# td-kwj-zp2023/webgpu-msm-bls12-377

Hardware: AMD Instinct MI355X
Metric: ms per 2^20 BLS12-377 G1 MSM (lower is better)
Workload: dtype u32 (29-bit limbs, 64-bit accumulate)

## Files before the change

webgpu-msm-bls12-377_amd/csrc/curves.hpp:

```cpp
#pragma once
#include <hip/hip_runtime.h>

#include "common.hpp"
#include "fp64_host.hpp"
#include "g1_xyzz.hpp"
#include "te377.hpp"

namespace msm377 {
namespace {


__device__ __forceinline__ void load_words16(const uint32_t* __restrict__ p, uint32_t* w, int nvec) {
  const uint4* s = reinterpret_cast<const uint4*>(p);
#pragma unroll
  for (int k = 0; k < nvec; k++) {
    uint4 v = s[k];
    w[4 * k + 0] = v.x;
    w[4 * k + 1] = v.y;
    w[4 * k + 2] = v.z;
    w[4 * k + 3] = v.w;
  }
}

struct G1Dev {
  static constexpr uint32_t REC_WORDS = 32;
  static constexpr bool HAS_QUAD = true;
  static constexpr uint32_t RAW_WORDS = 24;
  static constexpr uint32_t PT_WORDS = 52;
  static constexpr uint32_t COORD_WORDS = 16;
  static constexpr uint32_t BKT_WORDS = 4 * COORD_WORDS;
  static constexpr uint32_t OUT_WORDS = 48;
  static constexpr uint32_t RECORD_TAG = 0;
  static constexpr int MADD_PRODUCTS = 10;
  static constexpr int FORM_ID = MSM377_STAGE_FORM_XYZZ;
  using F = Fp;
  static constexpr uint32_t NL = 13, NW32 = 12;
  static __device__ __forceinline__ Fp::El to64() { return Fp::from_const(G1Consts::TO64); }
  using Base = G1Affine;
  using Pt = G1XYZZ;
  static __device__ __forceinline__ bool convert(const uint32_t* raw, uint32_t* rec) {
    Fp::El x = Fp::to_mont(Fp::from_words<12>(raw));
    Fp::El y = Fp::to_mont(Fp::from_words<12>(raw + 12));
#pragma unroll
    for (int j = 0; j < 13; j++) {
      rec[j] = x.l[j];
      rec[13 + j] = y.l[j];
    }
#pragma unroll
    for (int j = 26; j < 32; j++) rec[j] = 0;
    return false;
  }
  static __device__ __forceinline__ Base load_base(const uint32_t* __restrict__ bases, uint32_t idx) {
    uint32_t w[28];
    load_words16(bases + (size_t)idx * REC_WORDS, w, 7);
    Base p;
#pragma unroll
    for (int j = 0; j < 13; j++) {
      p.x.l[j] = w[j];
      p.y.l[j] = w[13 + j];
    }
    return p;
  }
  static __device__ __forceinline__ bool is_bad(const Pt&) { return false; }
  static __device__ __forceinline__ bool is_stored_identity(const Pt& p) { return G1::is_identity(p); }
  static __device__ __forceinline__ Pt identity() { return G1::identity(); }
  static __device__ __forceinline__ Pt madd(const Pt& a, const Base& q, bool negq) { return G1::madd(a, q, negq); }
  static __device__ __forceinline__ Pt first(const Base& q, bool negq) { return G1::madd(G1::identity(), q, negq); }
  static __device__ __forceinline__ Pt add(const Pt& a, const Pt& b) { return G1::add(a, b); }
  static __device__ __forceinline__ void to_words(const Pt& p, uint32_t* w) {
#pragma unroll
    for (int j = 0; j < 13; j++) {
      w[j] = p.x.l[j];
      w[13 + j] = p.y.l[j];
      w[26 + j] = p.zz.l[j];
      w[39 + j] = p.zzz.l[j];
    }
  }
  static __device__ __forceinline__ Pt from_words(const uint32_t* w) {
    Pt p;
#pragma unroll
    for (int j = 0; j < 13; j++) {
      p.x.l[j] = w[j];
      p.y.l[j] = w[13 + j];
      p.zz.l[j] = w[26 + j];
      p.zzz.l[j] = w[39 + j];
    }
    return p;
  }
};

struct EdDev {
  static constexpr uint32_t REC_WORDS = 32;
  static constexpr bool HAS_QUAD = true;
  static constexpr uint32_t RAW_WORDS = 16;
  static constexpr uint32_t PT_WORDS = 36;
  static constexpr uint32_t COORD_WORDS = 12;
  static constexpr uint32_t BKT_WORDS = 4 * COORD_WORDS;
  static constexpr uint32_t OUT_WORDS = 32;
  static constexpr uint32_t RECORD_TAG = 0;
  static constexpr int MADD_PRODUCTS = 7;
  static constexpr int FORM_ID = -1;
  using F = Fq;
  static constexpr uint32_t NL = 9, NW32 = 8;
  static __device__ __forceinline__ Fq::El to64() { return Fq::from_const(EdConsts::TO64); }
  using Base = EdLazy::ABase;
  using Pt = EdLazy::Ext;
  static __device__ __forceinline__ bool convert(const uint32_t* raw, uint32_t* rec) {
    Fq::El x = Fq::to_mont(Fq::from_words<8>(raw));
    Fq::El y = Fq::to_mont(Fq::from_words<8>(raw + 8));
    const Ed::Base b = Ed::make_base(x, y);
#pragma unroll
    for (int j = 0; j < 9; j++) {
      rec[j] = b.ymx.l[j];
      rec[9 + j] = b.ypx.l[j];
      rec[18 + j] = b.kt.l[j];
    }
#pragma unroll
    for (int j = 27; j < 32; j++) rec[j] = 0;
    return false;
  }
  static __device__ __forceinline__ Base load_base(const uint32_t* __restrict__ bases, uint32_t idx) {
    uint32_t w[28];
    load_words16(bases + (size_t)idx * REC_WORDS, w, 7);
    Base p;
#pragma unroll
    for (int j = 0; j < 9; j++) {
      p.ymx.l[j] = w[j];
      p.ypx.l[j] = w[9 + j];
      p.kt.l[j] = w[18 + j];
    }
    return p;
  }

  static __device__ __forceinline__ bool is_bad(const Pt&) { return false; }
  static __device__ __forceinline__ bool is_stored_identity(const Pt& p) { return Fq::is_zero(p.x) && Fq::eq(p.y, p.z); }
  static __device__ __forceinline__ Pt identity() { return EdLazy::identity(); }
  static __device__ __forceinline__ Pt madd(const Pt& a, const Base& q, bool negq) { return EdLazy::madd_affine(a, q, negq); }
  static __device__ __forceinline__ Pt first(const Base& q, bool negq) { return EdLazy::madd_affine(EdLazy::identity(), q, negq); }
  static __device__ __forceinline__ Pt add(const Pt& a, const Pt& b) { return EdLazy::add(a, b); }
  static __device__ __forceinline__ void to_words(const Pt& p, uint32_t* w) {
#pragma unroll
    for (int j = 0; j < 9; j++) {
      w[j] = p.x.l[j];
      w[9 + j] = p.y.l[j];
      w[18 + j] = p.t.l[j];
      w[27 + j] = p.z.l[j];
    }
  }
  static __device__ __forceinline__ Pt from_words(const uint32_t* w) {
    Pt p;
#pragma unroll
    for (int j = 0; j < 9; j++) {
      p.x.l[j] = w[j];
      p.y.l[j] = w[9 + j];
      p.t.l[j] = w[18 + j];
      p.z.l[j] = w[27 + j];
    }
    return p;
  }
};

struct TeDev {
  static constexpr uint32_t REC_WORDS = 64;
  static constexpr bool HAS_QUAD = true;
  static constexpr uint32_t RAW_WORDS = 24;
  static constexpr uint32_t PT_WORDS = 52;
  static constexpr uint32_t COORD_WORDS = 16;
  static constexpr uint32_t BKT_WORDS = 4 * COORD_WORDS;
  static constexpr uint32_t OUT_WORDS = 48;
  static constexpr uint32_t RECORD_TAG = TE_RECORD_TAG;
  static constexpr int MADD_PRODUCTS = 8;
  static constexpr int FORM_ID = MSM377_STAGE_FORM_TE;
  using F = Fp;
  static constexpr uint32_t NL = 13, NW32 = 12;
  static __device__ __forceinline__ Fp::El to64() { return Fp::from_const(G1Consts::TO64); }
  using Base = Te377::PBase;
  using Pt = Te377::Ext;
  using Pt_K = G1Consts;
  static __device__ __forceinline__ bool convert(const uint32_t* raw, uint32_t* rec) {
    const Base b = Te377::from_wire(raw, raw + 12, false);
#pragma unroll
    for (int j = 0; j < 13; j++) {
      rec[j] = b.ymx.l[j];
      rec[13 + j] = b.ypx.l[j];
      rec[26 + j] = b.kt.l[j];
      rec[39 + j] = b.z2.l[j];
    }
#pragma unroll
    for (int j = 52; j < 64; j++) rec[j] = 0;
    return Fp::is_zero(b.z2);
  }
  static __device__ __forceinline__ Base load_base(const uint32_t* __restrict__ bases, uint32_t idx) {
    uint32_t w[52];
    load_words16(bases + (size_t)idx * REC_WORDS, w, 13);
    Base p;
#pragma unroll
    for (int j = 0; j < 13; j++) {
      p.ymx.l[j] = w[j];
      p.ypx.l[j] = w[13 + j];
      p.kt.l[j] = w[26 + j];
      p.z2.l[j] = w[39 + j];
    }
    return p;
  }
  static __device__ __forceinline__ bool is_bad(const Pt& p) { return Te377::is_bad(p); }
  static __device__ __forceinline__ bool is_stored_identity(const Pt& p) { return Fp::is_zero(p.x) && Fp::eq(p.y, p.z); }
  static __device__ __forceinline__ Pt identity() { return Te377::identity(); }
  static __device__ __forceinline__ Pt madd(const Pt& a, const Base& q, bool negq) { return Te377::madd(a, q, negq); }
  static __device__ __forceinline__ Pt first(const Base& q, bool negq) { return Te377::from_base(q, negq); }
  static __device__ __forceinline__ Pt add(const Pt& a, const Pt& b) { return Te377::add(a, b); }
  static __device__ __forceinline__ void to_words(const Pt& p, uint32_t* w) {
#pragma unroll
    for (int j = 0; j < 13; j++) {
      w[j] = p.x.l[j];
      w[13 + j] = p.y.l[j];
      w[26 + j] = p.t.l[j];
      w[39 + j] = p.z.l[j];
    }
  }
  static __device__ __forceinline__ Pt from_words(const uint32_t* w) {
    Pt p;
#pragma unroll
    for (int j = 0; j < 13; j++) {
      p.x.l[j] = w[j];
      p.y.l[j] = w[13 + j];
      p.t.l[j] = w[26 + j];
      p.z.l[j] = w[39 + j];
    }
    return p;
  }
};

struct TeAffBase {
  static constexpr uint32_t REC_WORDS = 40;
  static constexpr int MADD_PRODUCTS = 7;
  using Base = Te377::ABase;
  using Pt = Te377::Ext;
  static __device__ __forceinline__ Base load_base(const uint32_t* __restrict__ bases, uint32_t idx) {
    uint32_t w[40];
    load_words16(bases + (size_t)idx * REC_WORDS, w, 10);
    Base p;
#pragma unroll
    for (int j = 0; j < 13; j++) {
      p.ymx.l[j] = w[j];
      p.ypx.l[j] = w[13 + j];
      p.kt.l[j] = w[26 + j];
    }
    return p;
  }
  static __device__ __forceinline__ Pt madd(const Pt& a, const Base& q, bool negq) { return Te377::madd_affine(a, q, negq); }
  static __device__ __forceinline__ Pt first(const Base& q, bool negq) { return Te377::from_base_affine(q, negq); }
};

template <class CV>
__device__ __forceinline__ typename CV::Pt load_record(const uint32_t* __restrict__ p) {
  uint32_t w[CV::PT_WORDS];
#pragma unroll
  for (uint32_t c = 0; c < 4; c++) {
    const uint4* s = reinterpret_cast<const uint4*>(p + c * CV::COORD_WORDS);
#pragma unroll
    for (uint32_t k = 0; k < CV::NL / 4; k++) {
      const uint4 v = s[k];
      w[c * CV::NL + 4 * k + 0] = v.x;
      w[c * CV::NL + 4 * k + 1] = v.y;
      w[c * CV::NL + 4 * k + 2] = v.z;
      w[c * CV::NL + 4 * k + 3] = v.w;
    }
    static_assert(CV::NL % 4 == 1, "one limb beyond the 16-byte groups");
    w[c * CV::NL + CV::NL - 1] = p[c * CV::COORD_WORDS + CV::NL - 1];
  }
  return CV::from_words(w);
}
template <class CV>
__device__ __forceinline__ void store_coord(uint32_t* __restrict__ slot, const uint32_t* l) {
  uint4* d = reinterpret_cast<uint4*>(slot);
#pragma unroll
  for (uint32_t k = 0; k < CV::NL / 4; k++) d[k] = make_uint4(l[4 * k], l[4 * k + 1], l[4 * k + 2], l[4 * k + 3]);
  d[CV::NL / 4] = make_uint4(l[CV::NL - 1], 0u, 0u, 0u);
  static_assert(CV::COORD_WORDS == (CV::NL / 4 + 1) * 4, "slot = limbs rounded up to 16 bytes");
}
template <class CV>
__device__ __forceinline__ void store_record(uint32_t* __restrict__ p, const typename CV::Pt& r) {
  uint32_t w[CV::PT_WORDS];
  CV::to_words(r, w);
#pragma unroll
  for (uint32_t c = 0; c < 4; c++) store_coord<CV>(p + c * CV::COORD_WORDS, w + c * CV::NL);
}
template <class CV>
__device__ __forceinline__ uint32_t* bucket_ptr(uint32_t* b, uint32_t L, uint32_t ws, uint32_t t) { return b + (((size_t)ws << L) + t) * CV::BKT_WORDS; }
template <class CV>
__device__ __forceinline__ const uint32_t* bucket_ptr(const uint32_t* b, uint32_t L, uint32_t ws, uint32_t t) { return b + (((size_t)ws << L) + t) * CV::BKT_WORDS; }
template <class CV>
__device__ __forceinline__ typename CV::Pt load_bucket(const uint32_t* __restrict__ b, uint32_t L, uint32_t ws, uint32_t t) {
  return load_record<CV>(bucket_ptr<CV>(b, L, ws, t));
}
template <class CV>
__device__ __forceinline__ void store_bucket(uint32_t* __restrict__ b, uint32_t L, uint32_t ws, uint32_t t, const typename CV::Pt& r) {
  store_record<CV>(bucket_ptr<CV>(b, L, ws, t), r);
}

static_assert(G1Dev::REC_WORDS == G1_REC_WORDS, "common.hpp sizes the base table with it");

}
}
```

webgpu-msm-bls12-377_amd/csrc/field29.hpp:

```cpp
#pragma once
#include <stdint.h>

#if defined(__HIPCC__)
#include <hip/hip_runtime.h>
#define MSM_HD __host__ __device__ __forceinline__
#else
#define MSM_HD inline __attribute__((always_inline))
#endif

#include "consts_gen.hpp"

namespace msm377 {

constexpr int LB = 29;
constexpr uint32_t LMASK = (1u << LB) - 1u;

template <int N>
struct Limbs {
  uint32_t l[N];
};

template <class C>
struct Field {
  static constexpr int N = C::NL;
  static constexpr int RS = C::RS;
  using Consts = C;
  using El = Limbs<N>;

  static MSM_HD El zero() {
    El r;
#pragma unroll
    for (int j = 0; j < N; j++) r.l[j] = 0;
    return r;
  }
  static MSM_HD El from_const(const uint32_t (&c)[N]) {
    El r;
#pragma unroll
    for (int j = 0; j < N; j++) r.l[j] = c[j];
    return r;
  }
  static MSM_HD El one() { return from_const(C::ONE); }

  static MSM_HD bool is_zero(const El& a) {
    uint32_t acc = 0;
#pragma unroll
    for (int j = 0; j < N; j++) acc |= a.l[j];
    return acc == 0;
  }
  static MSM_HD bool eq(const El& a, const El& b) {
    uint32_t acc = 0;
#pragma unroll
    for (int j = 0; j < N; j++) acc |= (a.l[j] ^ b.l[j]);
    return acc == 0;
  }
  static MSM_HD El select(bool c, const El& a, const El& b) {
    El r;
#pragma unroll
    for (int j = 0; j < N; j++) r.l[j] = c ? a.l[j] : b.l[j];
    return r;
  }

  static MSM_HD El reduce_once(const El& x) {
    El d;
    int32_t bw = 0;
#pragma unroll
    for (int j = 0; j < N - 1; j++) {
      int32_t v = (int32_t)x.l[j] - (int32_t)C::MOD[j] + bw;
      d.l[j] = (uint32_t)v & LMASK;
      bw = v >> 31;
    }
    int32_t top = (int32_t)x.l[N - 1] - (int32_t)C::MOD[N - 1] + bw;
    d.l[N - 1] = (uint32_t)top;
    return select(top < 0, x, d);
  }

  static MSM_HD El add(const El& a, const El& b) {
    El s;
    uint32_t c = 0;
#pragma unroll
    for (int j = 0; j < N - 1; j++) {
      uint32_t v = a.l[j] + b.l[j] + c;
      s.l[j] = v & LMASK;
      c = v >> LB;
    }
    s.l[N - 1] = a.l[N - 1] + b.l[N - 1] + c;
    return reduce_once(s);
  }
  static MSM_HD El dbl(const El& a) { return add(a, a); }

  static MSM_HD El sub(const El& a, const El& b) {
    El d, e;
    int32_t bw = 0, c2 = 0;
#pragma unroll
    for (int j = 0; j < N - 1; j++) {
      int32_t v = (int32_t)a.l[j] - (int32_t)b.l[j];
      int32_t v1 = v + bw;
      d.l[j] = (uint32_t)v1 & LMASK;
      bw = v1 >> 31;
      int32_t v2 = v + (int32_t)C::MOD[j] + c2;
      e.l[j] = (uint32_t)v2 & LMASK;
      c2 = v2 >> LB;
    }
    int32_t v = (int32_t)a.l[N - 1] - (int32_t)b.l[N - 1];
    int32_t top = v + bw;
    d.l[N - 1] = (uint32_t)top;
    e.l[N - 1] = (uint32_t)(v + (int32_t)C::MOD[N - 1] + c2);
    return select(top < 0, e, d);
  }

  static MSM_HD El neg(const El& a) {
    El r;
    int32_t bw = 0;
    uint32_t nz = 0;
#pragma unroll
    for (int j = 0; j < N; j++) {
      nz |= a.l[j];
      int32_t v = (int32_t)C::MOD[j] - (int32_t)a.l[j] + bw;
      r.l[j] = (j < N - 1) ? ((uint32_t)v & LMASK) : (uint32_t)v;
      bw = v >> 31;
    }
    return select(nz != 0, r, a);
  }
  static MSM_HD El cneg(const El& a, bool c) { return select(c, neg(a), a); }


  static MSM_HD El mul_lz(const El& a, const El& b) {
    uint64_t t[N];
#pragma unroll
    for (int j = 0; j < N; j++) t[j] = 0;
#pragma unroll
    for (int i = 0; i < RS; i++) {
      if (i < N) {
#pragma unroll
        for (int j = 0; j < N; j++) t[j] += (uint64_t)a.l[i] * b.l[j];
      }
      uint32_t q = (0u - (uint32_t)t[0]) & LMASK;
      uint64_t carry = (t[0] + q) >> LB;
#pragma unroll
      for (int j = 1; j < N; j++) t[j] += (uint64_t)q * C::MOD[j];
      t[1] += carry;
#pragma unroll
      for (int j = 0; j < N - 1; j++) t[j] = t[j + 1];
      t[N - 1] = 0;
    }
    El r;
#pragma unroll
    for (int j = 0; j < N - 1; j++) {
      r.l[j] = (uint32_t)t[j] & LMASK;
      t[j + 1] += t[j] >> LB;
    }
    r.l[N - 1] = (uint32_t)t[N - 1];
    return r;
  }

  static MSM_HD El mul_add_mul_lz(const El& a, const El& b, const El& e, const El& d) {
    uint64_t t[N];
#pragma unroll
    for (int j = 0; j < N; j++) t[j] = 0;
#pragma unroll
    for (int i = 0; i < RS; i++) {
      if (i < N) {
#pragma unroll
        for (int j = 0; j < N; j++) t[j] += (uint64_t)a.l[i] * b.l[j];
#pragma unroll
        for (int j = 0; j < N; j++) t[j] += (uint64_t)e.l[i] * d.l[j];
      }
      uint32_t q = (0u - (uint32_t)t[0]) & LMASK;
      uint64_t carry = (t[0] + q) >> LB;
#pragma unroll
      for (int j = 1; j < N; j++) t[j] += (uint64_t)q * C::MOD[j];
      t[1] += carry;
#pragma unroll
      for (int j = 0; j < N - 1; j++) t[j] = t[j + 1];
      t[N - 1] = 0;
    }
    El r;
#pragma unroll
    for (int j = 0; j < N - 1; j++) {
      r.l[j] = (uint32_t)t[j] & LMASK;
      t[j + 1] += t[j] >> LB;
    }
    r.l[N - 1] = (uint32_t)t[N - 1];
    return r;
  }

  static MSM_HD El sqr_lz(const El& a) {
    uint64_t t[RS + N];
#pragma unroll
    for (int j = 0; j < RS + N; j++) t[j] = 0;
#pragma unroll
    for (int i = 0; i < N; i++) {
      t[2 * i] += (uint64_t)a.l[i] * a.l[i];
      const uint32_t a2 = a.l[i] << 1;
#pragma unroll
      for (int j = i + 1; j < N; j++) t[i + j] += (uint64_t)a2 * a.l[j];
    }
#pragma unroll
    for (int i = 0; i < RS; i++) {
      uint32_t q = (0u - (uint32_t)t[i]) & LMASK;
      uint64_t carry = (t[i] + q) >> LB;
#pragma unroll
      for (int j = 1; j < N; j++) t[i + j] += (uint64_t)q * C::MOD[j];
      t[i + 1] += carry;
    }
    El r;
#pragma unroll
    for (int j = 0; j < N - 1; j++) {
      r.l[j] = (uint32_t)t[RS + j] & LMASK;
      t[RS + j + 1] += t[RS + j] >> LB;
    }
    r.l[N - 1] = (uint32_t)t[RS + N - 1];
    return r;
  }

  static MSM_HD El mul(const El& a, const El& b) { return reduce_once(mul_lz(a, b)); }
  static MSM_HD El sqr(const El& a) { return reduce_once(sqr_lz(a)); }
  static MSM_HD El mul_sub_mul(const El& a, const El& b, const El& c, const El& d) {
    const El r = mul_add_mul_lz(a, b, neg(c), d);
    return RS > N ? reduce_once(r) : reduce_once(reduce_once(r));
  }


  static MSM_HD El add_kp_sub(const El& a, const uint32_t (&K)[N], const El& b) {
    El r;
#pragma unroll
    for (int j = 0; j < N; j++) r.l[j] = a.l[j] + K[j] - b.l[j];
    return r;
  }
  static MSM_HD El add_lz(const El& a, const El& b) {
    El r;
#pragma unroll
    for (int j = 0; j < N; j++) r.l[j] = a.l[j] + b.l[j];
    return r;
  }
  static MSM_HD El kp_sub(const uint32_t (&K)[N], const El& b) {
    El r;
#pragma unroll
    for (int j = 0; j < N; j++) r.l[j] = K[j] - b.l[j];
    return r;
  }
  static MSM_HD El add_kp_sub_sub2(const El& a, const uint32_t (&K)[N], const El& b, const El& b2) {
    El r;
#pragma unroll
    for (int j = 0; j < N; j++) r.l[j] = a.l[j] + K[j] - b.l[j] - 2u * b2.l[j];
    return r;
  }
  static MSM_HD El norm(const El& a) {
    El r;
    uint32_t c = 0;
#pragma unroll
    for (int j = 0; j < N - 1; j++) {
      const uint32_t v = a.l[j] + c;
      r.l[j] = v & LMASK;
      c = v >> LB;
    }
    r.l[N - 1] = a.l[N - 1] + c;
    return r;
  }
  static MSM_HD El csub(const El& x, const uint32_t (&m)[N]) {
    El d;
    int32_t bw = 0;
#pragma unroll
    for (int j = 0; j < N - 1; j++) {
      const int32_t v = (int32_t)x.l[j] - (int32_t)m[j] + bw;
      d.l[j] = (uint32_t)v & LMASK;
      bw = v >> 31;
    }
    const int64_t top = (int64_t)x.l[N - 1] - (int64_t)m[N - 1] + bw;
    d.l[N - 1] = (uint32_t)top;
    return select(top < 0, x, d);
  }
  static MSM_HD El canon(const El& x) { return csub(csub(csub(x, C::MOD4), C::MOD2), C::MOD); }

  static MSM_HD El to_mont(const El& a) { return mul(a, from_const(C::R2)); }
  static MSM_HD El from_mont(const El& a) {
    El o = zero();
    o.l[0] = 1;
    return mul(a, o);
  }

  template <int NW>
  static MSM_HD El from_words(const uint32_t* w) {
    El r;
#pragma unroll
    for (int j = 0; j < N; j++) {
      const int bit = LB * j, wi = bit >> 5, off = bit & 31;
      uint32_t v = 0;
      if (wi < NW) v = w[wi] >> off;
      if (off > 32 - LB && wi + 1 < NW) v |= w[wi + 1] << (32 - off);
      r.l[j] = v & LMASK;
    }
    return r;
  }
  template <int NW>
  static MSM_HD void to_words(const El& a, uint32_t* w) {
#pragma unroll
    for (int k = 0; k < NW; k++) w[k] = 0;
#pragma unroll
    for (int j = 0; j < N; j++) {
      const int bit = LB * j, wi = bit >> 5, off = bit & 31;
      if (wi < NW) w[wi] |= a.l[j] << off;
      if (off > 32 - LB && wi + 1 < NW) w[wi + 1] |= a.l[j] >> (32 - off);
    }
  }
};

using Fp = Field<G1Consts>;
using Fq = Field<EdConsts>;

template <class F, int NW>
MSM_HD typename F::El fe_pow(const typename F::El& a, const uint32_t* e) {
  typename F::El r = F::one();
  for (int i = NW * 32 - 1; i >= 0; i--) {
    r = F::sqr(r);
    if ((e[i >> 5] >> (i & 31)) & 1u) r = F::mul(r, a);
  }
  return r;
}

}
```

webgpu-msm-bls12-377_amd/csrc/kernels/accumulate.hpp:

```cpp
#pragma once
#include "../curves.hpp"
#include "reduce.hpp"

namespace msm377 {
namespace {



__device__ __forceinline__ const uint32_t* row_bounds(const uint32_t* __restrict__ row_ptr, uint32_t L, uint32_t ws, uint32_t t) {
  return row_ptr + (size_t)ws * ((1u << L) + 2) + t + 1;
}
__device__ __forceinline__ uint32_t row_len(const uint32_t* __restrict__ row_ptr, uint32_t L, uint32_t row) {
  const int at = (int)(row + 2 * (row >> L) + 1);
  return row_ptr[at + 1] - row_ptr[at];
}

struct RowSplit {
  uint32_t nseg, seglen, lastlen;
};
__device__ __forceinline__ RowSplit row_split(uint32_t len, uint32_t SEG) {
  RowSplit r;
  if (len <= SEG) {
    r.nseg = 1;
    r.seglen = r.lastlen = len;
    return r;
  }
  const uint32_t parts = (len + SEG - 1) / SEG;
  r.seglen = (len + parts - 1) / parts;
  r.nseg = (len + r.seglen - 1) / r.seglen;
  r.lastlen = len - (r.nseg - 1) * r.seglen;
  return r;
}

__global__ void __launch_bounds__(1024) k_work_hist(const uint32_t* __restrict__ row_ptr, uint32_t L, uint32_t rows, uint32_t SEG, uint32_t* __restrict__ work_hist,
                                                   uint32_t* __restrict__ row_ovf_base, uint32_t* __restrict__ counters ,
                                                   uint32_t* __restrict__ split_rows) {
  __shared__ uint32_t lh[SEG_BINS];
  __shared__ uint32_t blk[4];
  const uint32_t tid = threadIdx.x, row = blockIdx.x * 1024 + tid;
  if (tid < SEG_BINS) lh[tid] = 0;
  if (tid < 2) blk[tid] = 0;
  __syncthreads();
  RowSplit sp = {1, 0, 0};
  uint32_t my_split = 0, my_ovf = 0;
  if (row < rows) {
    sp = row_split(row_len(row_ptr, L, row), SEG);
    atomicAdd(&lh[sp.lastlen], 1u);
    if (sp.nseg > 1) {
      atomicAdd(&lh[sp.seglen], sp.nseg - 1);
      my_split = atomicAdd(&blk[0], 1u);
      my_ovf = atomicAdd(&blk[1], sp.nseg - 1);
    }
  }
  __syncthreads();
  if (tid < SEG_BINS && lh[tid]) atomicAdd(&work_hist[tid], lh[tid]);
  if (tid == 0 && blk[0]) {
    blk[2] = atomicAdd(&counters[0], blk[0]);
    blk[3] = atomicAdd(&counters[1], blk[1]);
  }
  __syncthreads();
  if (sp.nseg > 1) {
    row_ovf_base[row] = blk[3] + my_ovf;
    split_rows[blk[2] + my_split] = row;
  }
}

__global__ void __launch_bounds__(1024) k_work_scatter(const uint32_t* __restrict__ row_ptr, uint32_t L, uint32_t rows, uint32_t SEG,
                                                      const uint32_t* __restrict__ work_hist, uint32_t* __restrict__ cursor, uint32_t* __restrict__ total,
                                                      WorkItem* __restrict__ work) {
  __shared__ uint32_t lh[SEG_BINS];
  __shared__ uint32_t lbase[SEG_BINS];
  __shared__ uint32_t gh[SEG_BINS];
  const uint32_t tid = threadIdx.x, row = blockIdx.x * 1024 + tid;
  if (tid < SEG_BINS) {
    lh[tid] = 0;
    gh[tid] = work_hist[tid];
  }
  __syncthreads();
  uint32_t first = 0;
  if (tid < SEG_BINS) {
    for (uint32_t b = tid + 1; b < SEG_BINS; b++) first += gh[b];
    if (tid == 0 && blockIdx.x == 0) *total = first + gh[0];
  }
  RowSplit sp = {0, 0, 0};
  uint32_t rank_full = 0, rank_last = 0;
  if (row < rows) {
    sp = row_split(row_len(row_ptr, L, row), SEG);
    if (sp.nseg > 1) rank_full = atomicAdd(&lh[sp.seglen], sp.nseg - 1);
    rank_last = atomicAdd(&lh[sp.lastlen], 1u);
  }
  __syncthreads();
  if (tid < SEG_BINS && lh[tid]) lbase[tid] = first + atomicAdd(&cursor[tid], lh[tid]);
  __syncthreads();
  if (row < rows) {
    for (uint32_t s = 0; s + 1 < sp.nseg; s++) work[lbase[sp.seglen] + rank_full + s] = WorkItem{row, s};
    work[lbase[sp.lastlen] + rank_last] = WorkItem{row, sp.nseg - 1};
  }
}

template <class CV, int OCC, class BP = CV, int PF = 0>
__global__ void __launch_bounds__(256, OCC) k_accumulate(const uint32_t* __restrict__ row_ptr, const uint32_t* __restrict__ val_idx,
                                                       const uint32_t* __restrict__ bases, uint32_t* __restrict__ buckets, uint64_t n,
                                                       const WorkItem* __restrict__ work, const uint32_t* __restrict__ work_total,
                                                       const uint32_t* __restrict__ row_ovf_base, uint32_t* __restrict__ ovf, uint32_t SEG,
                                                       int* __restrict__ err, const int* __restrict__ conv_err, uint32_t into, uint64_t table_stride, uint32_t L) {
  const uint32_t v = blockIdx.x * 256 + threadIdx.x;
  if (v == 0 && *conv_err) atomicOr(err, *conv_err);
  if (v >= *work_total) return;
  const WorkItem it = work[v];
  const uint32_t ws = it.row >> L, t = it.row & ((1u << L) - 1);
  const uint32_t* rb = row_bounds(row_ptr, L, ws, t);
  const uint32_t* vi = val_idx + (size_t)ws * n;
  bases += (size_t)ws * table_stride * BP::REC_WORDS;
  const uint32_t row_beg = rb[0], row_end = rb[1];
  const uint32_t seglen = row_split(row_end - row_beg, SEG).seglen;
  uint32_t k = row_beg + it.seg * seglen;
  const uint32_t end = (row_end - k > seglen) ? k + seglen : row_end;
  typename CV::Pt acc = (into && it.seg == 0) ? load_bucket<CV>(buckets, L, ws, t) : CV::identity();
  const bool start_fresh = !(into && it.seg == 0);
  bool bad = false;
  if (k < end) {
    typename BP::Base rec[PF + 1];
    uint32_t e[PF + 2];
#pragma unroll
    for (int j = 0; j <= PF + 1; j++) e[j] = (k + j < end) ? vi[k + j] : 0u;
#pragma unroll
    for (int j = 0; j <= PF; j++) rec[j] = BP::load_base(bases, e[j] & 0x7fffffffu);
    bool more = true;
    auto stage = [&](auto first_tag) {
      constexpr bool FIRST = decltype(first_tag)::value;
      k++;
      more = k < end;
      typename BP::Base fresh = rec[PF];
      uint32_t e_new = 0u;
      if (k + PF < end) {
        fresh = BP::load_base(bases, e[PF + 1] & 0x7fffffffu);
        if (k + PF + 1 < end) e_new = vi[k + PF + 1];
      }
      if constexpr (FIRST)
        acc = BP::first(rec[0], (e[0] >> 31) != 0);
      else
        acc = BP::madd(acc, rec[0], (e[0] >> 31) != 0);
      bad |= CV::is_bad(acc);
#pragma unroll
      for (int j = 0; j < PF; j++) rec[j] = rec[j + 1];
      rec[PF] = fresh;
#pragma unroll
      for (int j = 0; j <= PF; j++) e[j] = e[j + 1];
      e[PF + 1] = e_new;
    };
    if (start_fresh) stage(std::true_type{});
    while (more) stage(std::false_type{});
  }
  if (bad) atomicOr(err, ERR_TE_EXCEPTIONAL);
  if (it.seg == 0) {
    store_bucket<CV>(buckets, L, ws, t, acc);
  } else {
    store_record<CV>(ovf + (size_t)(row_ovf_base[it.row] + it.seg - 1) * CV::BKT_WORDS, acc);
  }
}

template <class F, class K>
__device__ __forceinline__ typename TeLazy<F, K>::Ext te_madd_quad(const typename TeLazy<F, K>::Ext& a, const typename F::El& mine, uint32_t q) {
  using El = typename F::El;
  const El m1 = F::mul_lz(sel4(q, F::add_kp_sub(a.y, K::KP2, a.x), F::add_lz(a.y, a.x), a.t, a.z), mine);
  const El pa = quad_bcast<0>(m1), pb = quad_bcast<1>(m1), c = quad_bcast<2>(m1), d = quad_bcast<3>(m1);
  const El e = F::norm(F::add_kp_sub(pb, K::KP2, pa)), f = F::norm(F::add_kp_sub(d, K::KP2, c));
  const El g = F::norm(F::add_lz(d, c)), h = F::add_lz(pb, pa);
  const El m3 = F::mul_lz(sel4(q, e, h, h, f), sel4(q, f, g, e, g));
  typename TeLazy<F, K>::Ext o;
  o.x = quad_bcast<0>(m3);
  o.y = quad_bcast<1>(m3);
  o.t = quad_bcast<2>(m3);
  o.z = quad_bcast<3>(m3);
  return o;
}

template <class CV>
__global__ void __launch_bounds__(256, 2) k_accumulate_quad(const uint32_t* __restrict__ row_ptr, const uint32_t* __restrict__ val_idx,
                                                          const uint32_t* __restrict__ bases, uint32_t* __restrict__ buckets, uint64_t n,
                                                          const WorkItem* __restrict__ work, const uint32_t* __restrict__ work_total,
                                                          const uint32_t* __restrict__ row_ovf_base, uint32_t* __restrict__ ovf, uint32_t SEG,
                                                          int* __restrict__ err, const int* __restrict__ conv_err, uint32_t into, uint32_t L) {
  using El = typename CV::F::El;
  using K = typename CV::Pt_K;
  const uint32_t gid = blockIdx.x * 256 + threadIdx.x;
  const uint32_t v = gid >> 2, q = threadIdx.x & 3;
  if (gid == 0 && *conv_err) atomicOr(err, *conv_err);
  if (v >= *work_total) return;
  const WorkItem it = work[v];
  const uint32_t ws = it.row >> L, t = it.row & ((1u << L) - 1);
  const uint32_t* rb = row_bounds(row_ptr, L, ws, t);
  const uint32_t* vi = val_idx + (size_t)ws * n;
  const uint32_t row_beg = rb[0], row_end = rb[1];
  const uint32_t seglen = row_split(row_end - row_beg, SEG).seglen;
  uint32_t k = row_beg + it.seg * seglen;
  const uint32_t end = (row_end - k > seglen) ? k + seglen : row_end;
  const bool continues = into && it.seg == 0;
  typename CV::Pt acc = continues ? load_bucket<CV>(buckets, L, ws, t) : CV::identity();
  bool bad = false;
  auto load_mine = [&](uint32_t e) {
    const bool neg = (e >> 31) != 0;
    const uint32_t comp = q < 2 ? (q ^ (neg ? 1u : 0u)) : q;
    const uint32_t* src = bases + (size_t)(e & 0x7fffffffu) * CV::REC_WORDS + comp * CV::NL;
    El r;
#pragma unroll
    for (int j = 0; j < (int)CV::NL; j++) r.l[j] = src[j];
    return r;
  };
  if (k < end && !continues) {
    const uint32_t e = vi[k];
    acc = CV::first(CV::load_base(bases, e & 0x7fffffffu), (e >> 31) != 0);
    bad |= CV::is_bad(acc);
    k++;
  }
  if (k < end) {
    uint32_t e_cur = vi[k];
    uint32_t e_nxt = (k + 1 < end) ? vi[k + 1] : 0u;
    El cur = load_mine(e_cur);
    for (;;) {
      k++;
      const bool more = k < end;
      El nxt = cur;
      uint32_t e_nn = 0u;
      if (more) {
        nxt = load_mine(e_nxt);
        if (k + 1 < end) e_nn = vi[k + 1];
      }
      const El mine = (q == 2 && (e_cur >> 31)) ? CV::F::kp_sub(K::KP2, cur) : cur;
      acc = te_madd_quad<typename CV::F, K>(acc, mine, q);
      bad |= CV::is_bad(acc);
      if (!more) break;
      cur = nxt;
      e_cur = e_nxt;
      e_nxt = e_nn;
    }
  }
  if (bad) atomicOr(err, ERR_TE_EXCEPTIONAL);
  uint32_t* dst = it.seg == 0 ? bucket_ptr<CV>(buckets, L, ws, t) : ovf + (size_t)(row_ovf_base[it.row] + it.seg - 1) * CV::BKT_WORDS;
  store_coord<CV>(dst + q * CV::COORD_WORDS, coord4(q, acc).l);
}

constexpr uint32_t OVF_FOLDED = 0x80000000u;
constexpr uint32_t LONG_ROW_PARTIALS = 32, FOLD_THREADS = 512, FOLD_BLOCKS = 64;
static_assert((1u << 15) <= FOLD_THREADS * FOLD_BLOCKS, "one pass of the grid sees every row of a window (L <= 15)");
template <class CV>
__global__ void __launch_bounds__(FOLD_THREADS) k_fold_long_rows(const uint32_t* __restrict__ row_ptr, uint32_t* __restrict__ row_ovf_base, uint32_t* __restrict__ ovf,
                                                                 uint32_t SEG, int* __restrict__ err, uint32_t L, uint32_t ws) {
  __shared__ uint32_t list[FOLD_THREADS];
  __shared__ uint32_t nlist;
  if (threadIdx.x == 0) nlist = 0;
  __syncthreads();
  {
    const uint32_t t = blockIdx.x + gridDim.x * threadIdx.x;
    if (t < (1u << L) && row_split(row_len(row_ptr, L, (ws << L) + t), SEG).nseg > LONG_ROW_PARTIALS) list[atomicAdd(&nlist, 1u)] = (ws << L) + t;
  }
  __syncthreads();
  const uint32_t q = threadIdx.x & 3, quad = threadIdx.x >> 2;
  bool bad = false;
  for (uint32_t i = 0; i < nlist; i++) {
    const uint32_t row = list[i];
    uint32_t* rec = ovf + (size_t)row_ovf_base[row] * CV::BKT_WORDS;
    for (uint32_t cur = row_split(row_len(row_ptr, L, row), SEG).nseg - 1; cur > 1;) {
      const uint32_t half = (cur + 1) / 2;
      for (uint32_t j = quad; j + half < cur; j += FOLD_THREADS / 4) {
        uint32_t* a = rec + (size_t)j * CV::BKT_WORDS;
        const typename CV::Pt sum = add_quad(load_record_quad<CV>(a, q), load_record_quad<CV>(rec + (size_t)(j + half) * CV::BKT_WORDS, q), q);
        bad |= CV::is_bad(sum);
        store_coord<CV>(a + q * CV::COORD_WORDS, coord4(q, sum).l);
      }
      cur = half;
      __syncthreads();
    }
  }
  __syncthreads();
  for (uint32_t i = threadIdx.x; i < nlist; i += FOLD_THREADS) row_ovf_base[list[i]] |= OVF_FOLDED;
  if (bad) atomicOr(err, ERR_TE_MERGE);
}

template <class CV>
__global__ void __launch_bounds__(256, 2) k_merge_split_rows_quad(const uint32_t* __restrict__ row_ptr, uint32_t* __restrict__ buckets,
                                                                  const uint32_t* __restrict__ counters, const uint32_t* __restrict__ split_rows,
                                                                  const uint32_t* __restrict__ row_ovf_base, const uint32_t* __restrict__ ovf, uint32_t SEG,
                                                                  int* __restrict__ err, uint32_t L, uint32_t* __restrict__ host_flag, uint32_t seq) {
  if (host_flag && blockIdx.x == 0 && threadIdx.x == 0) __hip_atomic_store(host_flag, seq, __ATOMIC_RELAXED, __HIP_MEMORY_SCOPE_SYSTEM);
  const uint32_t count = counters[0];
  const uint32_t q = threadIdx.x & 3;
  for (uint32_t i = (blockIdx.x * 256 + threadIdx.x) >> 2; i < count; i += gridDim.x * 64) {
    const uint32_t row = split_rows[i];
    const uint32_t len = row_len(row_ptr, L, row);
    const uint32_t ovf_at = row_ovf_base[row];
    const uint32_t nseg = (ovf_at & OVF_FOLDED) ? 2u : row_split(len, SEG).nseg;
    const uint32_t ws = row >> L, t = row & ((1u << L) - 1);
    typename CV::Pt acc = load_bucket_quad<CV>(buckets, L, ws, t, q);
    const uint32_t* src = ovf + (size_t)(ovf_at & ~OVF_FOLDED) * CV::BKT_WORDS;
    typename CV::Pt nxt = load_record_quad<CV>(src, q);
    bool bad = false;
    for (uint32_t s = 1; s < nseg; s++) {
      const typename CV::Pt cur = nxt;
      if (s + 1 < nseg) nxt = load_record_quad<CV>(src + (size_t)s * CV::BKT_WORDS, q);
      acc = add_quad(acc, cur, q);
      bad |= CV::is_bad(acc);
    }
    if (bad) atomicOr(err, ERR_TE_MERGE);
    const typename CV::F::El c = coord4(q, acc);
    store_coord<CV>(bucket_ptr<CV>(buckets, L, ws, t) + q * CV::COORD_WORDS, c.l);
  }
}

}
}
```

webgpu-msm-bls12-377_amd/csrc/te377.hpp:

```cpp
#pragma once
#include "ed_ext.hpp"
#include "field29.hpp"

namespace msm377 {

template <class F_, class K_>
struct TeLazy {
  using F = F_;
  using El = typename F::El;
  using K = K_;
  struct ABase {
    El ymx, ypx, kt;
  };
  struct PBase {
    El ymx, ypx, kt, z2;
  };
  struct Ext {
    El x, y, t, z;
  };
  static MSM_HD Ext identity() {
    Ext r;
    r.x = F::zero();
    r.y = F::one();
    r.t = F::zero();
    r.z = F::one();
    return r;
  }
  static MSM_HD bool is_zero_mod_p(const El& a) { return F::is_zero(a) || F::eq(a, F::from_const(K::MOD)); }
  static MSM_HD bool is_bad(const Ext& p) { return is_zero_mod_p(p.z); }

  static MSM_HD Ext madd(const Ext& p, const PBase& q, bool neg) {
    const El a = F::mul_lz(F::add_kp_sub(p.y, K::KP2, p.x), F::select(neg, q.ypx, q.ymx));
    const El b = F::mul_lz(F::add_lz(p.y, p.x), F::select(neg, q.ymx, q.ypx));
    const El c = F::mul_lz(F::select(neg, F::kp_sub(K::KP2, q.kt), q.kt), p.t);
    const El d = F::mul_lz(p.z, q.z2);
    return finish(a, b, c, d);
  }
  static MSM_HD Ext madd_affine(const Ext& p, const ABase& q, bool neg) {
    const El a = F::mul_lz(F::add_kp_sub(p.y, K::KP2, p.x), F::select(neg, q.ypx, q.ymx));
    const El b = F::mul_lz(F::add_lz(p.y, p.x), F::select(neg, q.ymx, q.ypx));
    const El c = F::mul_lz(F::select(neg, F::kp_sub(K::KP2, q.kt), q.kt), p.t);
    return finish(a, b, c, F::add_lz(p.z, p.z));
  }
  static MSM_HD Ext add(const Ext& p, const Ext& q) {
    const El a = F::mul_lz(F::norm(F::add_kp_sub(p.y, K::KP2, p.x)), F::norm(F::add_kp_sub(q.y, K::KP2, q.x)));
    const El b = F::mul_lz(F::norm(F::add_lz(p.y, p.x)), F::norm(F::add_lz(q.y, q.x)));
    const El c = F::mul_lz(F::mul_lz(p.t, q.t), F::from_const(K::TE_2D));
    const El d = F::mul_lz(p.z, q.z);
    return finish(a, b, c, F::add_lz(d, d));
  }
  static MSM_HD Ext finish(const El& a, const El& b, const El& c, const El& d) {
    const El e = F::norm(F::add_kp_sub(b, K::KP2, a));
    const El f = F::norm(F::add_kp_sub(d, K::KP2, c));
    const El g = F::norm(F::add_lz(d, c));
    const El h = F::add_lz(b, a);
    Ext r;
    r.x = F::mul_lz(e, f);
    r.y = F::mul_lz(h, g);
    r.t = F::mul_lz(h, e);
    r.z = F::mul_lz(f, g);
    return r;
  }
};

using EdLazy = TeLazy<Fq, EdConsts>;

struct Te377 : TeLazy<Fp, G1Consts> {
  using F = Fp;
  using El = Fp::El;
  using K = G1Consts;

  static MSM_HD PBase from_wire(const uint32_t* x12, const uint32_t* y12, bool phi) {
    const El xr = F::template from_words<12>(x12), yr = F::template from_words<12>(y12);
    const El u = F::add(F::mul(xr, F::from_const(phi ? K::TE_SBR : K::TE_SR)), F::from_const(K::TE_S));
    const El v = F::mul(yr, F::from_const(K::TE_SR));
    const El cu = F::add(F::mul(xr, F::from_const(phi ? K::TE_CSBR : K::TE_CSR)), F::from_const(K::TE_CS));
    const El up = F::add(u, F::one());
    const El X = F::mul(cu, up), Z = F::mul(v, up);
    const El T = F::sub(X, F::dbl(cu)), Y = F::sub(Z, F::dbl(v));
    PBase b;
    b.ymx = F::sub(Y, X);
    b.ypx = F::add(Y, X);
    b.kt = F::mul(T, F::from_const(K::TE_2D));
    b.z2 = F::dbl(Z);
    return b;
  }

  static MSM_HD Ext from_base(const PBase& q, bool neg) {
    Ext r;
    const El x2 = F::sub(q.ypx, q.ymx), t2 = F::mul(q.kt, F::from_const(K::TE_INV_D));
    r.x = F::cneg(x2, neg);
    r.y = F::add(q.ypx, q.ymx);
    r.t = F::cneg(t2, neg);
    r.z = q.z2;
    return r;
  }
  static MSM_HD Ext from_base_affine(const ABase& q, bool neg) {
    Ext r;
    const El x2 = F::sub(q.ypx, q.ymx), t2 = F::mul(q.kt, F::from_const(K::TE_INV_D));
    r.x = F::cneg(x2, neg);
    r.y = F::add(q.ypx, q.ymx);
    r.t = F::cneg(t2, neg);
    r.z = F::dbl(F::one());
    return r;
  }

  static MSM_HD ABase affine_from_wire(const uint32_t* x12, const uint32_t* y12, bool& bad) {
    const El xr = F::template from_words<12>(x12), yr = F::template from_words<12>(y12);
    const El u = F::add(F::mul(xr, F::from_const(K::TE_SR)), F::from_const(K::TE_S));
    const El v = F::mul(yr, F::from_const(K::TE_SR));
    const El cu = F::add(F::mul(xr, F::from_const(K::TE_CSR)), F::from_const(K::TE_CS));
    const El up = F::add(u, F::one()), um = F::sub(u, F::one());
    const El Z = F::mul(v, up);
    bad = F::is_zero(Z);
    const El zi = fe_pow<F, K::PM2_NW>(Z, K::PM2_W);
    const El x = F::mul(F::mul(cu, up), zi), y = F::mul(F::mul(um, v), zi);
    ABase b;
    b.ymx = F::sub(y, x);
    b.ypx = F::add(y, x);
    b.kt = F::mul(F::mul(x, y), F::from_const(K::TE_2D));
    return b;
  }

};

}
```

Before: 2.538.

## Precompute signed base operands, bias Montgomery columns, and wave-gate the bad-point check

The accumulate loop now resolves the sign-dependent selects and the negated kt into an operand struct before issuing the next base load, and pins those values in registers so the following load overlaps the madd. Montgomery multiplication pre-biases each column with LMASK, so the reduction digit becomes a single NOT-and-mask and the separate carry add is dropped. The Te377 bad-point check first tests limb 0 and uses a wave ballot to skip the full zero-mod-p comparison. In exchange the code holds more live registers, and the prefetch depth is fixed at one record.

```diff
diff --git a/webgpu-msm-bls12-377_amd/csrc/curves.hpp b/webgpu-msm-bls12-377_amd/csrc/curves.hpp
--- a/webgpu-msm-bls12-377_amd/csrc/curves.hpp
+++ b/webgpu-msm-bls12-377_amd/csrc/curves.hpp
@@ -65,6 +65,12 @@
   static __device__ __forceinline__ bool is_stored_identity(const Pt& p) { return G1::is_identity(p); }
   static __device__ __forceinline__ Pt identity() { return G1::identity(); }
   static __device__ __forceinline__ Pt madd(const Pt& a, const Base& q, bool negq) { return G1::madd(a, q, negq); }
+  struct Ops {
+    Base q;
+    uint32_t neg;
+  };
+  static __device__ __forceinline__ Ops signed_ops(const Base& q, bool negq) { return Ops{q, negq ? 1u : 0u}; }
+  static __device__ __forceinline__ Pt madd(const Pt& a, const Ops& o) { return G1::madd(a, o.q, o.neg != 0); }
   static __device__ __forceinline__ Pt first(const Base& q, bool negq) { return G1::madd(G1::identity(), q, negq); }
   static __device__ __forceinline__ Pt add(const Pt& a, const Pt& b) { return G1::add(a, b); }
   static __device__ __forceinline__ void to_words(const Pt& p, uint32_t* w) {
@@ -136,6 +142,9 @@
   static __device__ __forceinline__ bool is_stored_identity(const Pt& p) { return Fq::is_zero(p.x) && Fq::eq(p.y, p.z); }
   static __device__ __forceinline__ Pt identity() { return EdLazy::identity(); }
   static __device__ __forceinline__ Pt madd(const Pt& a, const Base& q, bool negq) { return EdLazy::madd_affine(a, q, negq); }
+  using Ops = EdLazy::AOps;
+  static __device__ __forceinline__ Ops signed_ops(const Base& q, bool negq) { return EdLazy::signed_ops(q, negq); }
+  static __device__ __forceinline__ Pt madd(const Pt& a, const Ops& o) { return EdLazy::madd_affine(a, o); }
   static __device__ __forceinline__ Pt first(const Base& q, bool negq) { return EdLazy::madd_affine(EdLazy::identity(), q, negq); }
   static __device__ __forceinline__ Pt add(const Pt& a, const Pt& b) { return EdLazy::add(a, b); }
   static __device__ __forceinline__ void to_words(const Pt& p, uint32_t* w) {
@@ -207,6 +216,9 @@
   static __device__ __forceinline__ bool is_stored_identity(const Pt& p) { return Fp::is_zero(p.x) && Fp::eq(p.y, p.z); }
   static __device__ __forceinline__ Pt identity() { return Te377::identity(); }
   static __device__ __forceinline__ Pt madd(const Pt& a, const Base& q, bool negq) { return Te377::madd(a, q, negq); }
+  using Ops = Te377::POps;
+  static __device__ __forceinline__ Ops signed_ops(const Base& q, bool negq) { return Te377::signed_ops(q, negq); }
+  static __device__ __forceinline__ Pt madd(const Pt& a, const Ops& o) { return Te377::madd(a, o); }
   static __device__ __forceinline__ Pt first(const Base& q, bool negq) { return Te377::from_base(q, negq); }
   static __device__ __forceinline__ Pt add(const Pt& a, const Pt& b) { return Te377::add(a, b); }
   static __device__ __forceinline__ void to_words(const Pt& p, uint32_t* w) {
@@ -249,6 +261,9 @@
     return p;
   }
   static __device__ __forceinline__ Pt madd(const Pt& a, const Base& q, bool negq) { return Te377::madd_affine(a, q, negq); }
+  using Ops = Te377::AOps;
+  static __device__ __forceinline__ Ops signed_ops(const Base& q, bool negq) { return Te377::signed_ops(q, negq); }
+  static __device__ __forceinline__ Pt madd(const Pt& a, const Ops& o) { return Te377::madd_affine(a, o); }
   static __device__ __forceinline__ Pt first(const Base& q, bool negq) { return Te377::from_base_affine(q, negq); }
 };
 
diff --git a/webgpu-msm-bls12-377_amd/csrc/field29.hpp b/webgpu-msm-bls12-377_amd/csrc/field29.hpp
--- a/webgpu-msm-bls12-377_amd/csrc/field29.hpp
+++ b/webgpu-msm-bls12-377_amd/csrc/field29.hpp
@@ -124,24 +124,33 @@
   static MSM_HD El cneg(const El& a, bool c) { return select(c, neg(a), a); }
 
 
+  static MSM_HD uint32_t mont_digit(uint64_t t0_biased) { return ~(uint32_t)t0_biased & LMASK; }
+  static MSM_HD uint64_t column_bias() {
+    uint64_t b = LMASK;
+#if defined(__HIP_DEVICE_COMPILE__)
+    asm("" : "+s"(b));
+#endif
+    return b;
+  }
+
   static MSM_HD El mul_lz(const El& a, const El& b) {
+    const uint64_t bias = column_bias();
     uint64_t t[N];
 #pragma unroll
-    for (int j = 0; j < N; j++) t[j] = 0;
+    for (int j = 0; j < N; j++) t[j] = bias;
 #pragma unroll
     for (int i = 0; i < RS; i++) {
       if (i < N) {
 #pragma unroll
         for (int j = 0; j < N; j++) t[j] += (uint64_t)a.l[i] * b.l[j];
       }
-      uint32_t q = (0u - (uint32_t)t[0]) & LMASK;
-      uint64_t carry = (t[0] + q) >> LB;
+      const uint32_t q = mont_digit(t[0]);
 #pragma unroll
       for (int j = 1; j < N; j++) t[j] += (uint64_t)q * C::MOD[j];
-      t[1] += carry;
+      t[1] += t[0] >> LB;
 #pragma unroll
       for (int j = 0; j < N - 1; j++) t[j] = t[j + 1];
-      t[N - 1] = 0;
+      t[N - 1] = (i + N < RS) ? bias : 0;
     }
     El r;
 #pragma unroll
@@ -154,9 +163,10 @@
   }
 
   static MSM_HD El mul_add_mul_lz(const El& a, const El& b, const El& e, const El& d) {
+    const uint64_t bias = column_bias();
     uint64_t t[N];
 #pragma unroll
-    for (int j = 0; j < N; j++) t[j] = 0;
+    for (int j = 0; j < N; j++) t[j] = bias;
 #pragma unroll
     for (int i = 0; i < RS; i++) {
       if (i < N) {
@@ -165,14 +175,13 @@
 #pragma unroll
         for (int j = 0; j < N; j++) t[j] += (uint64_t)e.l[i] * d.l[j];
       }
-      uint32_t q = (0u - (uint32_t)t[0]) & LMASK;
-      uint64_t carry = (t[0] + q) >> LB;
+      const uint32_t q = mont_digit(t[0]);
 #pragma unroll
       for (int j = 1; j < N; j++) t[j] += (uint64_t)q * C::MOD[j];
-      t[1] += carry;
+      t[1] += t[0] >> LB;
 #pragma unroll
       for (int j = 0; j < N - 1; j++) t[j] = t[j + 1];
-      t[N - 1] = 0;
+      t[N - 1] = (i + N < RS) ? bias : 0;
     }
     El r;
 #pragma unroll
@@ -185,9 +194,10 @@
   }
 
   static MSM_HD El sqr_lz(const El& a) {
+    const uint64_t bias = column_bias();
     uint64_t t[RS + N];
 #pragma unroll
-    for (int j = 0; j < RS + N; j++) t[j] = 0;
+    for (int j = 0; j < RS + N; j++) t[j] = (j < RS) ? bias : 0;
 #pragma unroll
     for (int i = 0; i < N; i++) {
       t[2 * i] += (uint64_t)a.l[i] * a.l[i];
@@ -197,11 +207,10 @@
     }
 #pragma unroll
     for (int i = 0; i < RS; i++) {
-      uint32_t q = (0u - (uint32_t)t[i]) & LMASK;
-      uint64_t carry = (t[i] + q) >> LB;
+      const uint32_t q = mont_digit(t[i]);
 #pragma unroll
       for (int j = 1; j < N; j++) t[i + j] += (uint64_t)q * C::MOD[j];
-      t[i + 1] += carry;
+      t[i + 1] += t[i] >> LB;
     }
     El r;
 #pragma unroll
diff --git a/webgpu-msm-bls12-377_amd/csrc/kernels/accumulate.hpp b/webgpu-msm-bls12-377_amd/csrc/kernels/accumulate.hpp
--- a/webgpu-msm-bls12-377_amd/csrc/kernels/accumulate.hpp
+++ b/webgpu-msm-bls12-377_amd/csrc/kernels/accumulate.hpp
@@ -96,6 +96,16 @@
     for (uint32_t s = 0; s + 1 < sp.nseg; s++) work[lbase[sp.seglen] + rank_full + s] = WorkItem{row, s};
     work[lbase[sp.lastlen] + rank_last] = WorkItem{row, sp.nseg - 1};
   }
+}
+
+template <class T>
+__device__ __forceinline__ void pin_registers(T& o) {
+  static_assert(sizeof(T) % 4 == 0, "whole words");
+  uint32_t w[sizeof(T) / 4];
+  __builtin_memcpy(w, &o, sizeof(T));
+#pragma unroll
+  for (int j = 0; j < (int)(sizeof(T) / 4); j++) asm volatile("" : "+v"(w[j]));
+  __builtin_memcpy(&o, w, sizeof(T));
 }
 
 template <class CV, int OCC, class BP = CV, int PF = 0>
@@ -120,34 +130,34 @@
   const bool start_fresh = !(into && it.seg == 0);
   bool bad = false;
   if (k < end) {
-    typename BP::Base rec[PF + 1];
-    uint32_t e[PF + 2];
-#pragma unroll
-    for (int j = 0; j <= PF + 1; j++) e[j] = (k + j < end) ? vi[k + j] : 0u;
-#pragma unroll
-    for (int j = 0; j <= PF; j++) rec[j] = BP::load_base(bases, e[j] & 0x7fffffffu);
+    static_assert(PF == 0, "one record in flight");
+    uint32_t e_cur = vi[k];
+    uint32_t e_nxt = (k + 1 < end) ? vi[k + 1] : 0u;
+    typename BP::Base rec = BP::load_base(bases, e_cur & 0x7fffffffu);
     bool more = true;
+    auto advance = [&]() {
+      k++;
+      more = k < end;
+      if (more) {
+        rec = BP::load_base(bases, e_nxt & 0x7fffffffu);
+        e_cur = e_nxt;
+        e_nxt = (k + 1 < end) ? vi[k + 1] : 0u;
+      }
+    };
     auto stage = [&](auto first_tag) {
       constexpr bool FIRST = decltype(first_tag)::value;
-      k++;
-      more = k < end;
-      typename BP::Base fresh = rec[PF];
-      uint32_t e_new = 0u;
-      if (k + PF < end) {
-        fresh = BP::load_base(bases, e[PF + 1] & 0x7fffffffu);
-        if (k + PF + 1 < end) e_new = vi[k + PF + 1];
+      const bool neg = (e_cur >> 31) != 0;
+      if constexpr (FIRST) {
+        const typename BP::Base cur = rec;
+        advance();
+        acc = BP::first(cur, neg);
+      } else {
+        typename BP::Ops ops = BP::signed_ops(rec, neg);
+        pin_registers(ops);
+        advance();
+        acc = BP::madd(acc, ops);
       }
-      if constexpr (FIRST)
-        acc = BP::first(rec[0], (e[0] >> 31) != 0);
-      else
-        acc = BP::madd(acc, rec[0], (e[0] >> 31) != 0);
       bad |= CV::is_bad(acc);
-#pragma unroll
-      for (int j = 0; j < PF; j++) rec[j] = rec[j + 1];
-      rec[PF] = fresh;
-#pragma unroll
-      for (int j = 0; j <= PF; j++) e[j] = e[j + 1];
-      e[PF + 1] = e_new;
     };
     if (start_fresh) stage(std::true_type{});
     while (more) stage(std::false_type{});
diff --git a/webgpu-msm-bls12-377_amd/csrc/te377.hpp b/webgpu-msm-bls12-377_amd/csrc/te377.hpp
--- a/webgpu-msm-bls12-377_amd/csrc/te377.hpp
+++ b/webgpu-msm-bls12-377_amd/csrc/te377.hpp
@@ -27,21 +27,52 @@
     return r;
   }
   static MSM_HD bool is_zero_mod_p(const El& a) { return F::is_zero(a) || F::eq(a, F::from_const(K::MOD)); }
-  static MSM_HD bool is_bad(const Ext& p) { return is_zero_mod_p(p.z); }
+  static MSM_HD bool is_bad(const Ext& p) {
+    const bool maybe = p.z.l[0] == 0 || p.z.l[0] == K::MOD[0];
+#if defined(__HIP_DEVICE_COMPILE__)
+    if (__builtin_amdgcn_ballot_w64(maybe) == 0) return false;
+#else
+    if (!maybe) return false;
+#endif
+    return is_zero_mod_p(p.z);
+  }
 
-  static MSM_HD Ext madd(const Ext& p, const PBase& q, bool neg) {
-    const El a = F::mul_lz(F::add_kp_sub(p.y, K::KP2, p.x), F::select(neg, q.ypx, q.ymx));
-    const El b = F::mul_lz(F::add_lz(p.y, p.x), F::select(neg, q.ymx, q.ypx));
-    const El c = F::mul_lz(F::select(neg, F::kp_sub(K::KP2, q.kt), q.kt), p.t);
+  struct AOps {
+    El fa, fb, fc;
+  };
+  struct POps {
+    El fa, fb, fc, z2;
+  };
+  static MSM_HD AOps signed_ops(const ABase& q, bool neg) {
+    AOps o;
+    o.fa = F::select(neg, q.ypx, q.ymx);
+    o.fb = F::select(neg, q.ymx, q.ypx);
+    o.fc = F::select(neg, F::kp_sub(K::KP2, q.kt), q.kt);
+    return o;
+  }
+  static MSM_HD POps signed_ops(const PBase& q, bool neg) {
+    POps o;
+    o.fa = F::select(neg, q.ypx, q.ymx);
+    o.fb = F::select(neg, q.ymx, q.ypx);
+    o.fc = F::select(neg, F::kp_sub(K::KP2, q.kt), q.kt);
+    o.z2 = q.z2;
+    return o;
+  }
+  static MSM_HD Ext madd(const Ext& p, const POps& q) {
+    const El a = F::mul_lz(F::add_kp_sub(p.y, K::KP2, p.x), q.fa);
+    const El b = F::mul_lz(F::add_lz(p.y, p.x), q.fb);
+    const El c = F::mul_lz(q.fc, p.t);
     const El d = F::mul_lz(p.z, q.z2);
     return finish(a, b, c, d);
   }
-  static MSM_HD Ext madd_affine(const Ext& p, const ABase& q, bool neg) {
-    const El a = F::mul_lz(F::add_kp_sub(p.y, K::KP2, p.x), F::select(neg, q.ypx, q.ymx));
-    const El b = F::mul_lz(F::add_lz(p.y, p.x), F::select(neg, q.ymx, q.ypx));
-    const El c = F::mul_lz(F::select(neg, F::kp_sub(K::KP2, q.kt), q.kt), p.t);
+  static MSM_HD Ext madd(const Ext& p, const PBase& q, bool neg) { return madd(p, signed_ops(q, neg)); }
+  static MSM_HD Ext madd_affine(const Ext& p, const AOps& q) {
+    const El a = F::mul_lz(F::add_kp_sub(p.y, K::KP2, p.x), q.fa);
+    const El b = F::mul_lz(F::add_lz(p.y, p.x), q.fb);
+    const El c = F::mul_lz(q.fc, p.t);
     return finish(a, b, c, F::add_lz(p.z, p.z));
   }
+  static MSM_HD Ext madd_affine(const Ext& p, const ABase& q, bool neg) { return madd_affine(p, signed_ops(q, neg)); }
   static MSM_HD Ext add(const Ext& p, const Ext& q) {
     const El a = F::mul_lz(F::norm(F::add_kp_sub(p.y, K::KP2, p.x)), F::norm(F::add_kp_sub(q.y, K::KP2, q.x)));
     const El b = F::mul_lz(F::norm(F::add_lz(p.y, p.x)), F::norm(F::add_lz(q.y, q.x)));
```

Measured after the change: 2.410 (median of 6 runs). 5.0% less time.
